# outofforest/storm

Measured on AMD Instinct MI355X. Metric: GiB/s device-resident block checksum; % of MI355X HBM roofline, higher is better.
Workload: dtype u64

## Files before the change

storm_amd/csrc/commit_plan.h:

```cpp
#pragma once

#include <algorithm>
#include <atomic>
#include <cstdint>
#include <cstdlib>
#include <cstring>
#include <memory>
#include <vector>

#include "../../include/stormck.h"
#include "dispatch.h"

namespace stormck {

constexpr unsigned kMaxParts = 16;

enum class CommitError { Ok, TooMany, ParentRange, OriginAlign, Cycle, NoMem };

inline const char* commit_error_message(CommitError e) {
    switch (e) {
        case CommitError::TooMany: return "more than 2^32 dirty blocks";
        case CommitError::ParentRange: return "parent index out of range";
        case CommitError::OriginAlign: return "origin_pointer must be 8-byte aligned (Go blocks.Pointer alignment)";
        case CommitError::Cycle: return "parent links form a cycle";
// ... 193 lines not shown
    for (unsigned t = 1; t < parts; ++t)
        for (size_t l = 1; l <= max_h; ++l) pos[t][l] = pos[t - 1][l] + hist[t - 1][l];
    par(nu, [&](unsigned t, uint64_t lo, uint64_t hi) {
        std::vector<uint64_t>& ps = pos[t];
        for (uint64_t u = lo; u < hi; ++u) {
            const uint32_t i = uidx(u);
            O->order[ps[height[i]]++] = i;
        }
    });
}

template <class Par>
void commit_order(const Heights& H, Par&& par, CommitOrder* O) {
    order_level0(H, par, O);
    order_upper(H, par, O);
}

template <class Par, class Emit>
void relocate_range(stormck_dirty_block* blocks, const CommitOrder& O, uint64_t a, uint64_t b, uint64_t revision,
                    bool relocating, uint64_t* last, Par&& par, Emit&& emit) {
    if (a >= b) return;
    uint64_t before[kMaxParts + 1];
    before[0] = 0;
    unsigned parts = 0;
    if (relocating) {
        parts = par(b - a, [&](unsigned t, uint64_t lo, uint64_t hi) {
            uint64_t m = 0;
            for (uint64_t k = a + lo; k < a + hi; ++k) m += blocks[O.at(k)].birth_revision <= revision;
            before[t + 1] = m;
        });
        for (unsigned t = 0; t < parts; ++t) before[t + 1] += before[t];
    }
    const uint64_t first = *last;
    par(b - a, [&](unsigned t, uint64_t lo, uint64_t hi) {
        uint64_t addr = first + (relocating ? before[t] : 0);
        for (uint64_t k = a + lo; k < a + hi; ++k) {
            stormck_dirty_block& rec = blocks[O.at(k)];
            if (relocating && rec.birth_revision <= revision) {
                rec.address = ++addr;
                rec.birth_revision = revision + 1;
            }
            emit(k, rec);
        }
    });
    *last = first + before[parts];
}

constexpr uint64_t level0_chunk(uint64_t rest, uint64_t next) {
    return rest - std::min(next, rest) < kStreamBatch ? rest : std::min(next, rest);
}

constexpr bool commit_one_piece(uint64_t nu, uint64_t n0) { return nu > 0 && n0 <= kCommitOnePiece; }

}
```

storm_amd/csrc/dispatch.h:

```cpp
#pragma once

#include <algorithm>
#include <cstdint>
#include <cstdio>
#include <cstdlib>

#include "../../include/stormck.h"

namespace stormck {

constexpr int kU = 16;
constexpr int kQuadSpreadDepth = 4;
constexpr int kTileStripes = 16;
constexpr int kRing = 2;
constexpr int kGldsWaves = 8;
constexpr unsigned kGldsThreads = 64 * kGldsWaves;
constexpr unsigned kGldsBlocks = 16 * kGldsWaves;
constexpr int kAuxNT = 2;
constexpr uint64_t kMultiBpw = 5;
constexpr uint64_t kMultiBpwRing = 8;
constexpr uint64_t kMultiBpwWide = 16;
constexpr uint32_t kChunkPiecesWide = 128;
constexpr uint64_t kWideBatch = 128;
constexpr uint64_t kCommitWide = 256;
// ... 3 lines not shown
constexpr uint64_t kBigW = 131072;
constexpr uint64_t kBigBatch = 24576;
constexpr int kMidWaves = 2;
constexpr unsigned kThreads = 256;
constexpr uint32_t kMaxFanout = 1u << 16;
constexpr uint64_t kWideNodes = 256;
constexpr uint32_t kRingTile = 15;
constexpr int kRingPrefetch = 6;

constexpr int kSkewTiles = 8;
constexpr uint64_t kSkewMinSteps = 3584;

constexpr uint64_t kVarMinLen = 4096;
constexpr uint64_t kOrderMinBlocks = 1u << 20;

constexpr uint64_t kVarFloorPerCu = 44;
constexpr uint64_t kMidFloorPerCu = 36;
constexpr uint64_t kCommitFloorPerCu = 39;
constexpr uint64_t kAssumedCus = 256;

constexpr uint32_t kPlanRingSlots = 4;
constexpr uint64_t kPlanPipePieces = 4096;
constexpr uint64_t kPlanMultiPieces = 2034;
constexpr uint32_t kPlanOrderBuckets = 4096;
constexpr uint32_t kPlanNodeLds = 32768;
constexpr uint32_t plan_pointer_block_size(uint32_t fanout) { return (fanout * 25u + 7u) & ~7u; }

#ifdef STORMCK_PROBES
constexpr bool kProbes = true;
#else
constexpr bool kProbes = false;
#endif

struct Knobs {
    uint32_t ring_slots = kPlanRingSlots;
    bool wide16 = false;
    bool wide_multi = true;
    bool glds_var = true;
    uint64_t var_lo = 0;
    uint64_t var_min_len = kVarMinLen;
    int mid_waves = 0;
    bool big_w = true;
    uint64_t skew_min_steps = kSkewMinSteps;
    uint64_t quad_spread = 1;
    bool gather_order = true;
    bool gather_rank = false;
    bool gather_defer = false;
    bool order_idx = false;
    bool gather_contig = false;
    uint64_t commit_wide = kCommitWide;
    bool commit_multi = true;
    bool commit_midw = true;
    uint64_t commit_first = 2 * kStreamBatch, commit_growth = 3;
    int pointer_ring = 2;
    int pointer_c = 1;
    bool pointer_simd = true;
    uint64_t single_gpu_min = UINT64_MAX;
};

#ifdef STORMCK_PROBES
inline const Knobs& knobs() {
    static const Knobs once = [] {
        Knobs k;
        auto env = [](const char* name) { return std::getenv(name); };
        auto is = [&](const char* name, char c) { return env(name) && env(name)[0] == c; };
        auto num = [&](const char* name, uint64_t dflt) { return env(name) ? std::strtoull(env(name), nullptr, 10) : dflt; };
        auto integer = [&](const char* name, int dflt) { return env(name) ? std::atoi(env(name)) : dflt; };
        if (is("STORMCK_STAGE_PIPE", '0')) k.ring_slots = 0;
        k.wide16 = is("STORMCK_WIDE16", '1');
        k.wide_multi = !is("STORMCK_WIDE_MULTI", '0');
        k.glds_var = !is("STORMCK_GLDS_VAR", '0');
        k.var_lo = num("STORMCK_VAR_LO", 0);
        k.var_min_len = num("STORMCK_VAR_MIN_LEN", kVarMinLen);
        k.mid_waves = integer("STORMCK_MID_WAVES", 0);
        k.big_w = !is("STORMCK_BIG_W", '0');
        k.skew_min_steps = num("STORMCK_SKEW_MIN_STEPS", kSkewMinSteps);
        k.quad_spread = static_cast<uint64_t>(integer("STORMCK_QUAD_SPREAD", 1));
        k.gather_order = !is("STORMCK_GATHER_ORDER", '0');
        k.gather_rank = is("STORMCK_GATHER_RANK", '1');
        k.gather_defer = is("STORMCK_GATHER_DEFER", '1');
        k.order_idx = is("STORMCK_ORDER_IDX", '1');
        k.gather_contig = is("STORMCK_GATHER_CONTIG", '1');
        k.commit_multi = !is("STORMCK_COMMIT_MULTI", '0');
        k.commit_midw = !is("STORMCK_COMMIT_MIDW", '0');
        k.pointer_ring = integer("STORMCK_POINTER_RING", 2);
        k.pointer_c = integer("STORMCK_POINTER_C", 1);
        k.pointer_simd = !is("STORMCK_POINTER_SIMD", '0');
        k.single_gpu_min = num("STORMCK_SINGLE_GPU_MIN", UINT64_MAX);
        return k;
    }();
    return once;
}
inline Knobs commit_knobs() {
    Knobs k = knobs();
    if (const char* e = std::getenv("STORMCK_COMMIT_WIDE")) k.commit_wide = std::strtoull(e, nullptr, 10);
    unsigned long long f = 0, gr = 0;
    if (const char* e = std::getenv("STORMCK_COMMIT_CHUNKS"))
        if (std::sscanf(e, "%llu,%llu", &f, &gr) == 2 && f >= 1 && gr >= 1) {
            k.commit_first = f;
            k.commit_growth = gr;
        }
    return k;
}
#else
constexpr Knobs knobs() { return Knobs{}; }
constexpr Knobs commit_knobs() { return Knobs{}; }
#endif

enum class Kernel {
    Wide,
    WideMulti,
    GldsVar,
    GldsVarOrdered,
    Glds,
    GldsSkew,
    QuadSpread,
    Quad,
    PointerPc,
    TooLarge,
};

struct MultiShape {
    uint64_t bpw = 0;
    uint32_t ring = 0, chunk = 256;
    bool dbl = false;
};

struct Plan {
    Kernel kernel = Kernel::Quad;
    uint32_t grid = 0, block = kThreads;
    int waves = 0;
    bool persistent = false;
    bool simd_roles = false;
    MultiShape multi;
    uint64_t ws_bytes = 0;
    bool defer = false, idx = false, rank = false, contig = false;
};

inline Plan make_plan(Kernel k, uint64_t grid, unsigned block, int waves = 0) {
    Plan p;
    p.kernel = grid > 0x7fffffffULL ? Kernel::TooLarge : k;
    p.grid = static_cast<uint32_t>(grid);
    p.block = block;
    p.waves = waves;
    return p;
}

constexpr uint64_t busiest_cu_blocks(uint64_t n, uint64_t waves, uint64_t ncu) {
    return (((n + 16 * waves - 1) / (16 * waves)) + ncu - 1) / ncu * 16 * waves;
}
constexpr int mid_waves_for(uint64_t n, uint64_t ncu) {
    return busiest_cu_blocks(n, 1, ncu) < busiest_cu_blocks(n, 3, ncu) ? 1 : 3;
}
constexpr bool big_takes_3_waves(uint64_t n, uint64_t ncu) {
// ... 56 lines not shown
            p.rank = q.lens && persistent && k.gather_rank && n / kGldsBlocks > 0;
            p.contig = persistent && k.gather_contig;
            const uint64_t words = (uint64_t{kPlanOrderBuckets} * 3 + n + 1) & ~uint64_t{1};
            p.ws_bytes = words * 4 + n * 8 + (q.lens ? n * 4 : 0) + (p.defer ? n * 8 + 8 : 0);
        }
        return p;
    }
    int mid_waves = 0;
    if (ncu > 0 && n < kBigBatch) {
        if (k.mid_waves >= 1 && k.mid_waves <= 4) {
            if (n > 16 * ncu) mid_waves = k.mid_waves;
        } else if (k.mid_waves == 0 && n >= kMidFloorPerCu * ncu) {
            mid_waves = mid_waves_for(n, ncu);
        }
    } else if (ncu > 0 && n < kBigW && k.mid_waves == 0 && k.big_w) {
        if (big_takes_3_waves(n, ncu)) mid_waves = 3;
    }
    const bool streamable = !q.lens && !q.offs && rows16 && q.len >= 32u * kTileStripes;
    if (mid_waves > 0 && streamable)
        return make_plan(Kernel::Glds, (n + 16 * mid_waves - 1) / (16 * mid_waves), 64u * mid_waves, mid_waves);
    if (n >= kMidBatch && streamable) {
        if (n < kBigBatch)
            return make_plan(Kernel::Glds, (n + 16 * kMidWaves - 1) / (16 * kMidWaves), 64u * kMidWaves, kMidWaves);
        const uint64_t wgs = (n + kGldsBlocks - 1) / kGldsBlocks;
        if (wgs > 0x7fffffffULL) return make_plan(Kernel::TooLarge, 0, 0);
        if (ncu > 0 && wgs >= ncu && (wgs + ncu - 1) / ncu * ((q.len / 32) / kTileStripes) >= k.skew_min_steps)
            return make_plan(Kernel::GldsSkew, ncu, kGldsThreads, kGldsWaves);
        return make_plan(Kernel::Glds, wgs, kGldsThreads, kGldsWaves);
    }
    if (ncu > 0 && n <= 16 * k.quad_spread * ncu) return make_plan(Kernel::QuadSpread, (n + 15) / 16, 64);
    const uint64_t wgs = (n * 4 + kThreads - 1) / kThreads;
    return make_plan(wgs == 0 ? Kernel::TooLarge : Kernel::Quad, wgs, kThreads);
}

inline Plan plan_commit_level(uint64_t cnt, uint64_t ncu, bool glds_levels, const Knobs& k) {
    if (k.commit_midw && glds_levels && ncu > 0 && cnt >= kCommitFloorPerCu * ncu &&
        (cnt < kBigBatch || (cnt < kBigW && k.big_w && big_takes_3_waves(cnt, ncu)))) {
        const int w = cnt < kBigBatch ? mid_waves_for(cnt, ncu) : 3;
        return make_plan(Kernel::Glds, (cnt + 16 * w - 1) / (16 * w), 64u * w, w);
    }
    if (glds_levels && cnt >= kStreamBatch)
        return make_plan(Kernel::Glds, (cnt + kGldsBlocks - 1) / kGldsBlocks, kGldsThreads, kGldsWaves);
    if (cnt <= k.commit_wide) return make_plan(Kernel::Wide, cnt, kThreads);
    const MultiShape ms = multi_shape(cnt, ncu, k);
    if (k.commit_multi && ms.bpw > 0) {
        Plan p = make_plan(Kernel::WideMulti, (cnt + ms.bpw - 1) / ms.bpw, kThreads);
        p.multi = ms;
        return p;
    }
    const uint64_t wgs = (cnt * 4 + kThreads - 1) / kThreads;
    return make_plan(wgs == 0 ? Kernel::TooLarge : Kernel::Quad, wgs, kThreads);
}

inline Plan plan_pointer_level(uint64_t pm, uint32_t fanout, uint64_t ncu, const Knobs& k) {
    if (pm <= kWideNodes && plan_pointer_block_size(fanout) <= kPlanNodeLds) return make_plan(Kernel::Wide, pm, kThreads);
    if (k.pointer_ring != 0 && fanout == STORMCK_POINTERS_PER_BLOCK) {
        const uint64_t chains = (pm + 15) / 16, cus = ncu ? ncu : kAssumedCus;
        const int c = k.pointer_c == 1 || k.pointer_c == 2 || k.pointer_c == 4 ? k.pointer_c
                      : chains <= cus ? 1 : chains <= 2 * cus ? 2 : 4;
        Plan p = make_plan(Kernel::PointerPc, (chains + c - 1) / c, 128u * c, c);
        p.simd_roles = c > 1 && k.pointer_simd;
        return p;
    }
    const uint64_t wgs = (pm * 4 + kThreads - 1) / kThreads;
    return make_plan(wgs == 0 ? Kernel::TooLarge : Kernel::Quad, wgs, kThreads);
}

constexpr uint32_t kKeysPerWave = 8;
constexpr int kKeyRing = 4;
struct KeyTagsPlan {
    bool too_large = false;
    uint64_t batches = 0;
    int pieces = 0;
    bool fixed_len = false;
    uint32_t grid = 0, lds = 0;
    uint64_t tail = 0;
    uint32_t tail_grid = 0;
};

inline KeyTagsPlan plan_key_tags(uint64_t stride, uint32_t len, uint64_t n, bool offs, bool lens, unsigned base_low4) {
    KeyTagsPlan p;
    auto grid_for = [&](uint64_t threads, uint32_t* grid) {
        const uint64_t wgs = (threads + kThreads - 1) / kThreads;
        *grid = static_cast<uint32_t>(wgs);
        if (wgs == 0 || wgs > 0x7fffffffULL) p.too_large = true;
    };
    p.tail = n;
    grid_for(n, &p.tail_grid);
    if (p.too_large) return p;
    if (!offs && !lens && stride >= 16 && stride <= 256 && (stride & 15) == 0 && len <= stride && base_low4 == 0 && n >= 64) {
        p.batches = n / 64;
        p.pieces = static_cast<int>(stride / 16);
        p.fixed_len = len == stride;
        const uint64_t waves = (p.batches + kKeysPerWave - 1) / kKeysPerWave;
        p.grid = static_cast<uint32_t>((waves + 3) / 4);
        p.lds = static_cast<uint32_t>(4 * (p.pieces <= 4 ? kKeyRing : 2) * 64 * stride);
        p.tail = n - p.batches * 64;
        if (p.tail) grid_for(p.tail, &p.tail_grid);
    }
    return p;
}

}
```

storm_amd/csrc/kernels.h:

```cpp
#pragma once
#include "../../include/stormck.h"
#include "xxh64_dev.h"

namespace stormck {

typedef unsigned long long u64x2 __attribute__((ext_vector_type(2)));

#ifdef STORMCK_DEBUG_QUAD
__device__ unsigned long long g_partial_quads;
#endif

template <int K>
__device__ __forceinline__ uint64_t quad_bcast(uint64_t v) {
#ifdef STORMCK_DEBUG_QUAD
    {
        const uint64_t exec = __builtin_amdgcn_read_exec();
        const uint32_t quad = __lane_id() & ~3u;
        if (((exec >> quad) & 0xFull) != 0xFull) atomicAdd(&g_partial_quads, 1ull);
    }
#endif
    constexpr int ctrl = K | (K << 2) | (K << 4) | (K << 6);
    const int lo = __builtin_amdgcn_update_dpp(0, static_cast<int>(static_cast<uint32_t>(v)), ctrl, 0xF, 0xF, false);
    const int hi = __builtin_amdgcn_update_dpp(0, static_cast<int>(static_cast<uint32_t>(v >> 32)), ctrl, 0xF, 0xF, false);
    return (static_cast<uint64_t>(static_cast<uint32_t>(hi)) << 32) | static_cast<uint32_t>(lo);
// ... 1829 lines not shown
        out_cs[lo + first + b] = h;
        if (r.origin_pointer != STORMCK_NO_ORIGIN) {
            uint64_t* p = reinterpret_cast<uint64_t*>(arena + r.origin_pointer);
            p[0] = h;
            p[1] = r.address;
            p[2] = r.birth_revision;
            arena[r.origin_type] = r.type;
        }
    };
    if constexpr (RING > 0) {
        __shared__ uint4 ring[BPW * ring_block_pieces(RING, CP) + kRingSlackPieces];
        __shared__ uint32_t ready[pipe_max_chunks(CP)], done[1], abort_w[1];
        const PipeCtl pc{ready, done, abort_w, fault, kFaultCommitMulti, stall};
        multi_stage_hash_pipe<BPW, RING, CP, DBL>(ring, pc, nlive, src_of, emit, [](uint32_t) {});
    } else {
        __shared__ uint4 buf[BPW * kMultiPieces];
        multi_stage_hash<BPW>(buf, nlive, src_of, emit);
    }
}

template <int U>
__global__ __launch_bounds__(256) void k_commit_level(uint8_t* __restrict__ arena,
                                                       const stormck_dirty_block* __restrict__ blocks, uint64_t lo,
                                                       uint64_t cnt, uint64_t* __restrict__ out_cs) {
    const uint64_t gtid = static_cast<uint64_t>(blockIdx.x) * 256 + threadIdx.x;
    const uint64_t k = gtid >> 2;
    const uint32_t j = threadIdx.x & 3;
    const bool live = k < cnt;
    const uint64_t kk = live ? k : cnt - 1;
    const stormck_dirty_block b = blocks[lo + kk];
    const uint8_t* src = arena + b.data_offset;
    const uint32_t L = b.length;
    const uint32_t nst = L >> 5;
    uint64_t acc = acc_seed(j);
    if ((reinterpret_cast<uintptr_t>(src) & 7) == 0)
        acc = quad_stripes_aligned<U>(reinterpret_cast<const uint64_t*>(src) + j, nst, acc);
    else
        acc = quad_stripes_unaligned(src + 8 * j, nst, acc);
    const uint64_t v1 = quad_bcast<0>(acc), v2 = quad_bcast<1>(acc), v3 = quad_bcast<2>(acc), v4 = quad_bcast<3>(acc);
    if (j == 0 && live) {
        const uint64_t h0 = (L >= 32) ? converge(v1, v2, v3, v4) : kP5;
        const uint64_t h = finish_fast(h0, L, src + 32 * static_cast<uint64_t>(nst), L & 31);
        out_cs[lo + kk] = h;
        if (b.origin_pointer != STORMCK_NO_ORIGIN) {
            uint64_t* p = reinterpret_cast<uint64_t*>(arena + b.origin_pointer);
            p[0] = h;
            p[1] = b.address;
            p[2] = b.birth_revision;
            arena[b.origin_type] = b.type;
        }
    }
}

template <int T, int AUX, int WAVES>
__global__ __launch_bounds__(64 * WAVES) void k_commit_level_glds(uint8_t* __restrict__ arena,
                                                                   const stormck_dirty_block* __restrict__ blocks,
                                                                   uint64_t lo, uint64_t cnt,
                                                                   uint64_t* __restrict__ out_cs) {
    constexpr int R = 2;
    constexpr int BPW = 16 * WAVES;
    constexpr int ROW = 32 * T;
    constexpr int TILE = BPW * ROW;
    constexpr int INSTR = TILE / 1024;
    constexpr int PER_WAVE = INSTR / WAVES;
    constexpr int RW = sizeof(stormck_dirty_block) / 8;
    static_assert(INSTR % WAVES == 0, "tile must split evenly over the waves");
    __shared__ __attribute__((aligned(16))) uint8_t lds[R * TILE];
    uint64_t* rec_lds = reinterpret_cast<uint64_t*>(lds + TILE);
    static_assert(BPW * RW * 8 <= TILE, "records fit in one ring slot");

    const uint32_t tid = threadIdx.x;
    const uint32_t wave = tid >> 6, lane = tid & 63;
    const uint64_t k0 = static_cast<uint64_t>(blockIdx.x) * BPW;
    const uint32_t nrec = static_cast<uint32_t>(min<uint64_t>(BPW, cnt - k0));
    {
        const uint64_t* src = reinterpret_cast<const uint64_t*>(blocks + lo + k0);
        uint64_t w[(BPW * RW + 64 * WAVES - 1) / (64 * WAVES)];
#pragma unroll
        for (int m = 0; m < (BPW * RW + 64 * WAVES - 1) / (64 * WAVES); ++m) {
            const uint32_t q = tid + m * 64 * WAVES;
            w[m] = q < nrec * RW ? src[q] : 0;
        }
#pragma unroll
        for (int m = 0; m < (BPW * RW + 64 * WAVES - 1) / (64 * WAVES); ++m) {
            const uint32_t q = tid + m * 64 * WAVES;
            if (q < BPW * RW) rec_lds[q] = w[m];
        }
    }
    __syncthreads();
    const stormck_dirty_block* recs = reinterpret_cast<const stormck_dirty_block*>(rec_lds);

    const uint8_t* src[PER_WAVE];
    uint32_t ntl[PER_WAVE];
#pragma unroll
    for (int k = 0; k < PER_WAVE; ++k) {
        const uint32_t ii = wave * PER_WAVE + k;
        const uint32_t off = ii * 1024 + lane * 16;
        const uint32_t bb = off / ROW, q = (off % ROW) / 16;
        const uint32_t piece = (q + glds_rot<T>(bb)) % (2 * T);
        const bool plive = bb < nrec;
        const stormck_dirty_block& r = recs[plive ? bb : 0];
        src[k] = arena + r.data_offset + piece * 16;
        ntl[k] = plive ? (r.length >> 5) / T : 0;
    }
    const uint32_t b = tid >> 2, j = tid & 3;
    const uint64_t kb = k0 + b;
    const bool live = b < nrec;
    const stormck_dirty_block rec = recs[live ? b : 0];
    const uint32_t L = rec.length, nst = L >> 5;
    const uint32_t my_tiles = live ? nst / T : 0;
    uint32_t wg_tiles = my_tiles;
#pragma unroll
    for (int m = 32; m >= 1; m >>= 1) wg_tiles = max(wg_tiles, static_cast<uint32_t>(__shfl_xor(static_cast<int>(wg_tiles), m)));
    uint32_t* red = reinterpret_cast<uint32_t*>(lds);
    if (lane == 0) red[wave] = wg_tiles;
    __syncthreads();
    wg_tiles = 0;
    for (int w = 0; w < WAVES; ++w) wg_tiles = max(wg_tiles, red[w]);
    __syncthreads();

    const uint32_t rot = glds_rot<T>(b);
    uint64_t acc = acc_seed(j);
#if defined(__HIP_DEVICE_COMPILE__)
#define STORMCK_GLDS_ISSUE_MASKED(T_, SLOT)                                                              \
    do {                                                                                              \
        uint8_t* dst_ = lds + (SLOT) * TILE + wave * PER_WAVE * 1024;                                \
        _Pragma("unroll") for (int k_ = 0; k_ < PER_WAVE; ++k_) if ((T_) < ntl[k_])                   \
            __builtin_amdgcn_global_load_lds(src[k_] + static_cast<uint64_t>(T_) * ROW, dst_ + k_ * 1024, \
                                             16, 0, AUX);                                             \
    } while (0)
#else
#define STORMCK_GLDS_ISSUE_MASKED(T_, SLOT) do { } while (0)
#endif
    if (wg_tiles > 0) STORMCK_GLDS_ISSUE_MASKED(0u, 0);
    for (uint32_t t = 0; t < wg_tiles; ++t) {
        wait_vmcnt<0>();
        __builtin_amdgcn_s_barrier();
        if (t + 1 < wg_tiles) STORMCK_GLDS_ISSUE_MASKED(t + 1, (t + 1) & 1);
        if (t < my_tiles) {
            const uint8_t* row = lds + (t & 1) * TILE + b * ROW + (j & 1) * 8;
#pragma unroll
            for (int s = 0; s < T; ++s) {
                const uint32_t q = (2 * s + (j >> 1) + 2 * T - rot) % (2 * T);
                acc = round(acc, *reinterpret_cast<const uint64_t*>(row + q * 16));
            }
        }
    }
#undef STORMCK_GLDS_ISSUE_MASKED
    const uint8_t* bsrc = arena + rec.data_offset;
    for (uint32_t s = my_tiles * T; s < nst; ++s) acc = round(acc, reinterpret_cast<const uint64_t*>(bsrc)[4 * s + j]);
    const uint64_t v1 = quad_bcast<0>(acc), v2 = quad_bcast<1>(acc), v3 = quad_bcast<2>(acc), v4 = quad_bcast<3>(acc);
    if (j == 0 && live) {
        const uint64_t h0 = (L >= 32) ? converge(v1, v2, v3, v4) : kP5;
        const uint64_t h = finish_fast(h0, L, bsrc + 32 * static_cast<uint64_t>(nst), L & 31);
        out_cs[lo + kb] = h;
        if (rec.origin_pointer != STORMCK_NO_ORIGIN) {
            uint64_t* p = reinterpret_cast<uint64_t*>(arena + rec.origin_pointer);
            p[0] = h;
            p[1] = rec.address;
            p[2] = rec.birth_revision;
            arena[rec.origin_type] = rec.type;
        }
    }
}

__device__ __forceinline__ uint64_t ld64_any(const uint8_t* p, bool aligned) {
    return aligned ? *reinterpret_cast<const uint64_t*>(p) : ld64_unaligned(p);
}

template <bool OFFS, bool LENS>
__global__ __launch_bounds__(256) void k_key_tags(const uint8_t* __restrict__ keys, uint64_t stride,
                                                   const uint64_t* __restrict__ offs, const uint32_t* __restrict__ lens,
                                                   uint32_t len, uint64_t n, uint64_t* __restrict__ out) {
    const uint64_t i = static_cast<uint64_t>(blockIdx.x) * 256 + threadIdx.x;
    if (i >= n) return;
    const uint8_t* p = keys + (OFFS ? offs[i] : i * stride);
    const uint32_t L = LENS ? lens[i] : len;
    const bool al = (reinterpret_cast<uintptr_t>(p) & 7) == 0;
    const uint32_t nst = L >> 5;
    uint64_t h;
    if (L >= 32) {
        uint64_t v1 = kV1, v2 = kV2, v3 = kV3, v4 = kV4;
        for (uint32_t s = 0; s < nst; ++s) {
            const uint8_t* q = p + 32 * s;
            v1 = round(v1, ld64_any(q, al));
            v2 = round(v2, ld64_any(q + 8, al));
            v3 = round(v3, ld64_any(q + 16, al));
            v4 = round(v4, ld64_any(q + 24, al));
        }
        h = converge(v1, v2, v3, v4);
    } else {
        h = kP5;
    }
    out[i] = finish_fast(h, L, p + 32 * nst, L & 31);
}

template <int AUX, int P, int RING, int PW, int KLEN = 0, int SM = 0>
__global__ __launch_bounds__(256) void k_key_tags_ring(const uint8_t* __restrict__ keys, uint32_t len_rt,
                                                        uint64_t batches, uint64_t* __restrict__ out) {
    static_assert(RING >= 2 && PW >= RING, "ring");
    static_assert(KLEN >= 0 && KLEN <= 16 * P, "key length within the stride");
    const uint32_t len = KLEN > 0 ? static_cast<uint32_t>(KLEN) : len_rt;
    constexpr uint32_t kStride = 16 * P, kRegion = 64 * kStride;
    extern __shared__ __attribute__((aligned(16))) uint8_t dyn_lds[];
    const uint32_t wave = threadIdx.x >> 6, lane = threadIdx.x & 63;
    uint8_t* buf = dyn_lds + wave * RING * kRegion;
    const uint64_t b0 = (static_cast<uint64_t>(blockIdx.x) * 4 + wave) * PW;
    if (b0 >= batches) return;
    const uint32_t nb = static_cast<uint32_t>(batches - b0 < PW ? batches - b0 : PW);
    const uint32_t nst = len >> 5, rem = len & 31;
#if defined(__HIP_DEVICE_COMPILE__)
#define STORMCK_RING_ISSUE(I)                                                                              \
    do {                                                                                                  \
        const uint8_t* s_ = keys + (b0 + (I)) * kRegion + lane * 16;                                      \
        uint8_t* d_ = buf + ((I) % RING) * kRegion;                                                       \
        _Pragma("unroll") for (int p_ = 0; p_ < P; ++p_)                                                  \
// ... 145 lines not shown
```

storm_amd/csrc/stormck.hip:

```cpp
#include <hip/hip_runtime.h>

#include <algorithm>
#include <chrono>
#include <cstdlib>
#include <atomic>
#include <condition_variable>
#include <cstdio>
#include <cstring>
#include <memory>
#include <mutex>
#include <string>
#include <system_error>
#include <functional>
#include <thread>
#include <type_traits>
#include <vector>

#include <dlfcn.h>
#include <fcntl.h>
#include <pthread.h>
#include <sched.h>
#include <sys/uio.h>
#include <unistd.h>

// ... 518 lines not shown
        t0 = last = std::chrono::steady_clock::now();
    }
    void mark(const char* phase) {
        if (!on) return;
        const auto now = std::chrono::steady_clock::now();
        char buf[96];
        std::snprintf(buf, sizeof buf, " %s=%.3fms", phase, std::chrono::duration<double, std::milli>(now - last).count());
        log += buf;
        last = now;
    }
    ~PhaseTimer() {
        if (!on) return;
        const auto now = std::chrono::steady_clock::now();
        std::fprintf(stderr, "[stormck] %s total=%.3fms%s\n", what,
                     std::chrono::duration<double, std::milli>(now - t0).count(), log.c_str());
    }
};

__global__ void k_init_result(uint64_t* r, uint64_t n) {
    if (threadIdx.x == 0) {
        r[0] = n;
        r[1] = 0;
    }
}

constexpr uint64_t kChunkBytes = 256ULL << 20;
constexpr int kStages = 2;

struct Stage {
    hipStream_t stream = nullptr;
    hipEvent_t done = nullptr;
    hipEvent_t ready = nullptr;
    uint8_t* pinned = nullptr;
    uint8_t* d_data = nullptr;
    uint32_t* d_lens = nullptr;
    uint64_t* d_offs = nullptr;
    uint64_t* d_out = nullptr;
    uint64_t* h_out = nullptr;
    uint64_t* d_expected = nullptr;
    uint64_t* d_result = nullptr;
    uint64_t* h_result = nullptr;
    uint64_t first = 0, count = 0;
    bool busy = false;
};

struct DeviceCtx {
    std::mutex mu;
    int device = -1;
    bool ready = false;
    Stage st[kStages];
    stormck_dirty_block* commit_rec = nullptr;
    uint64_t* commit_cs = nullptr;
    uint64_t commit_n = 0;
};

std::mutex g_ctx_mu;
std::vector<std::unique_ptr<DeviceCtx>> g_ctx;

int get_ctx(DeviceCtx** out) {
    int rc = device_check();
    if (rc) return rc;
    int dev = 0;
    HIP_TRY(hipGetDevice(&dev));
    rc = fault_table_ready(dev);
    if (rc) return rc;
    std::lock_guard<std::mutex> g(g_ctx_mu);
    if (g_ctx.size() <= static_cast<size_t>(dev)) g_ctx.resize(dev + 1);
    if (!g_ctx[dev]) {
        g_ctx[dev].reset(new DeviceCtx());
        g_ctx[dev]->device = dev;
    }
    *out = g_ctx[dev].get();
    return STORMCK_OK;
}

int ensure_ready(DeviceCtx* c) {
    if (c->ready) return STORMCK_OK;
    for (Stage& s : c->st) {
        HIP_TRY(hipStreamCreateWithFlags(&s.stream, hipStreamNonBlocking));
        HIP_TRY(hipEventCreateWithFlags(&s.done, hipEventDisableTiming));
        HIP_TRY(hipEventCreateWithFlags(&s.ready, hipEventDisableTiming | hipEventBlockingSync));
        HIP_TRY(hipHostMalloc(reinterpret_cast<void**>(&s.pinned), kChunkBytes, hipHostMallocDefault));
        HIP_TRY(hipMalloc(&s.d_data, kChunkBytes));
        const uint64_t maxb = kChunkBytes / 8;
        HIP_TRY(hipMalloc(&s.d_lens, maxb * 4));
        HIP_TRY(hipMalloc(&s.d_offs, maxb * 8));
        HIP_TRY(hipMalloc(&s.d_out, maxb * 8));
        HIP_TRY(hipMalloc(&s.d_expected, maxb * 8));
        HIP_TRY(hipHostMalloc(reinterpret_cast<void**>(&s.h_out), maxb * 8, hipHostMallocDefault));
        HIP_TRY(hipMalloc(&s.d_result, 16));
        HIP_TRY(hipHostMalloc(reinterpret_cast<void**>(&s.h_result), 16, hipHostMallocDefault));
    }
    c->ready = true;
    return STORMCK_OK;
}

void release_ctx(DeviceCtx* c) {
    if (!c || (!c->ready && !c->commit_rec)) return;
    int prev = 0;
    (void)hipGetDevice(&prev);
    (void)hipSetDevice(c->device);
    for (Stage& s : c->st) {
        if (s.stream) (void)hipStreamSynchronize(s.stream);
        (void)hipFree(s.d_data);
        (void)hipFree(s.d_lens);
        (void)hipFree(s.d_offs);
        (void)hipFree(s.d_out);
        (void)hipFree(s.d_expected);
        (void)hipFree(s.d_result);
        (void)hipHostFree(s.pinned);
        (void)hipHostFree(s.h_out);
        (void)hipHostFree(s.h_result);
        if (s.done) (void)hipEventDestroy(s.done);
        if (s.ready) (void)hipEventDestroy(s.ready);
        if (s.stream) (void)hipStreamDestroy(s.stream);
        s = Stage();
    }
    c->ready = false;
    if (c->commit_rec) (void)hipHostFree(c->commit_rec);
    if (c->commit_cs) (void)hipHostFree(c->commit_cs);
    c->commit_rec = nullptr;
    c->commit_cs = nullptr;
    c->commit_n = 0;
    (void)hipSetDevice(prev);
}

bool host_readable(const void* p, uint64_t bytes) {
    const uint8_t* b = static_cast<const uint8_t*>(p);
    uint8_t got[2];
    iovec local = {got, 2};
    iovec remote[2] = {{const_cast<uint8_t*>(b), 1}, {const_cast<uint8_t*>(b + (bytes ? bytes - 1 : 0)), 1}};
    const ssize_t r = process_vm_readv(getpid(), &local, 1, remote, 2, 0);
    if (r == 2) return true;
    if (r >= 0 || errno == EFAULT) return false;
    static std::mutex mu;
    static int fds[2] = {-1, -1};
    std::lock_guard<std::mutex> g(mu);
    if (fds[0] < 0 && pipe2(fds, O_NONBLOCK | O_CLOEXEC) != 0) return true;
    for (const uint8_t* q : {b, b + (bytes ? bytes - 1 : 0)}) {
        if (write(fds[1], q, 1) != 1) return errno != EFAULT;
        uint8_t sink = 0;
        (void)!read(fds[0], &sink, 1);
    }
    return true;
}

enum class Mem {
    kPageable,
    kPinned,
    kMapped,
    kDevice,
    kUnreadable,
};
constexpr int kRegSlots = 16;
std::mutex g_reg_mu;
std::atomic<uintptr_t> g_reg_lo[kRegSlots], g_reg_hi[kRegSlots];
std::atomic<int> g_reg_n{0};

bool in_registered(const void* p, uint64_t bytes) {
    const int n = g_reg_n.load(std::memory_order_acquire);
    const uintptr_t x = reinterpret_cast<uintptr_t>(p);
    for (int k = 0; k < n; ++k) {
        const uintptr_t lo = g_reg_lo[k].load(std::memory_order_acquire);
        const uintptr_t hi = g_reg_hi[k].load(std::memory_order_acquire);
        if (lo && x >= lo && x < hi && bytes <= hi - x) return true;
    }
    return false;
}

void reg_add(void* p, uint64_t bytes) {
    std::lock_guard<std::mutex> g(g_reg_mu);
    for (int k = 0; k < kRegSlots; ++k)
        if (g_reg_lo[k].load(std::memory_order_relaxed) == 0) {
            g_reg_hi[k].store(reinterpret_cast<uintptr_t>(p) + bytes, std::memory_order_release);
            g_reg_lo[k].store(reinterpret_cast<uintptr_t>(p), std::memory_order_release);
            if (k >= g_reg_n.load(std::memory_order_relaxed)) g_reg_n.store(k + 1, std::memory_order_release);
// ... 941 lines not shown
        if (p.pieces <= 4)
            with_int<1, 2, 3, 4>(p.pieces, [&](auto P) {
                with_consts([&](auto FIXED) {
                    hipLaunchKernelGGL((k_key_tags_ring<kAuxNT, STORMCK_V(P), kKeyRing, kKeysPerWave,
                                                        STORMCK_V(FIXED) ? 16 * STORMCK_V(P) : 0, kKeyStore>),
                                       dim3(p.grid), dim3(kThreads), p.lds, st, k, len, p.batches, d_out);
                }, p.fixed_len);
            });
        else
            hipLaunchKernelGGL(k_key_tags_lds<kAuxNT>, dim3(p.grid), dim3(kThreads), p.lds, st, k,
                               static_cast<uint32_t>(stride), len, p.batches, kKeysPerWave, d_out);
        HIP_TRY(hipGetLastError());
        if (p.tail == 0) return STORMCK_OK;
        k += p.batches * 64 * stride;
        d_out += p.batches * 64;
    }
    with_consts([&](auto OFFS, auto LENS) {
        hipLaunchKernelGGL((k_key_tags<STORMCK_V(OFFS), STORMCK_V(LENS)>), dim3(p.tail_grid), dim3(kThreads), 0, st, k, stride,
                           d_offsets, d_lens, len, p.tail, d_out);
    }, d_offsets != nullptr, d_lens != nullptr);
    HIP_TRY(hipGetLastError());
    return STORMCK_OK;
}


}

namespace {

struct PoolPar {
    unsigned cap;
    uint64_t grain;
    template <class F>
    unsigned operator()(uint64_t count, F&& fn) const {
        if (cap <= 1 || count < grain) {
            fn(0u, uint64_t{0}, count);
            return 1;
        }
        ForkJoin& fj = ForkJoin::get();
        const unsigned nt = static_cast<unsigned>(std::min<uint64_t>({cap, kMaxParts, fj.size(), count / grain + 1}));
        fj.run(nt, [&](unsigned t) { fn(t, count * t / nt, count * (t + 1) / nt); });
        return nt;
    }
};
PoolPar plan_par(uint32_t threads = 0) { return {threads ? threads : kMaxParts, 16384}; }
PoolPar stage_par(uint32_t threads = 0) { return {threads ? std::min(threads, 8u) : 8u, 8192}; }

int commit_forest(const stormck_dirty_block* blocks, uint64_t n, uint64_t revision, uint32_t threads, Heights* H) {
    const CommitError e = commit_heights(blocks, n, revision, plan_par(threads), H);
    if (e == CommitError::Ok) return STORMCK_OK;
    return fail(e == CommitError::NoMem ? STORMCK_ENOMEM : STORMCK_EINVAL, commit_error_message(e));
}

int commit_device_run(void* d_arena, stormck_dirty_block* blocks, const Heights& H, uint64_t revision,
                      uint64_t* last_allocated_block, uint64_t* out_checksums, void* stream, PhaseTimer& pt) {
    ForkJoin& fj = ForkJoin::get();
    const uint64_t n = H.n, nu = H.n_upper, n0 = H.n0();
    const bool glds_levels =
        (reinterpret_cast<uintptr_t>(d_arena) & 15) == 0 && !H.data_off16 && H.longest > knobs().var_min_len;

    DeviceCtx* c = nullptr;
    int rc = get_ctx(&c);
    if (rc) return rc;
    std::lock_guard<std::mutex> g(c->mu);
    rc = ensure_ready(c);
    if (rc) return rc;
    if (c->commit_n < n) {
        if (c->commit_rec) (void)hipHostFree(c->commit_rec);
        if (c->commit_cs) (void)hipHostFree(c->commit_cs);
        c->commit_rec = nullptr;
        c->commit_cs = nullptr;
        c->commit_n = 0;
        HIP_TRY(hipHostMalloc(reinterpret_cast<void**>(&c->commit_rec), n * sizeof(stormck_dirty_block),
                              hipHostMallocCoherent));
        HIP_TRY(hipHostMalloc(reinterpret_cast<void**>(&c->commit_cs), n * 8, hipHostMallocCoherent));
        c->commit_n = n;
    }
    stormck_dirty_block* d_blocks = nullptr;
    uint64_t* d_cs = nullptr;
    HIP_TRY(hipHostGetDevicePointer(reinterpret_cast<void**>(&d_blocks), c->commit_rec, 0));
    HIP_TRY(hipHostGetDevicePointer(reinterpret_cast<void**>(&d_cs), c->commit_cs, 0));
    pt.mark("ctx");

    CommitOrder O;
    if (!H.prefix0()) {
        order_level0(H, plan_par(), &O);
        pt.mark("order0");
    }
    const std::vector<uint32_t>& order = O.order;

    hipStream_t st = static_cast<hipStream_t>(stream);
    const Knobs kn = commit_knobs();
    const uint64_t ncu = cu_count();
    uint8_t* arena = static_cast<uint8_t*>(d_arena);
    auto launch_level = [&](uint64_t lo, uint64_t cnt) -> int {
        const Plan p = plan_commit_level(cnt, ncu, glds_levels, kn);
        const dim3 grid(p.grid), block(p.block);
        switch (p.kernel) {
            case Kernel::TooLarge:
                return fail(STORMCK_EINVAL, "level too large");
            case Kernel::Glds:
                with_int<1, 3, kGldsWaves>(p.waves, [&](auto W) {
                    hipLaunchKernelGGL((k_commit_level_glds<kTileStripes, kAuxNT, STORMCK_V(W)>), grid, block, 0, st, arena,
                                       d_blocks, lo, cnt, d_cs);
                });
                break;
            case Kernel::Wide:
                hipLaunchKernelGGL(k_commit_level_wide, grid, block, 0, st, arena, d_blocks, lo, d_cs);
                break;
            case Kernel::WideMulti: {
                const int mrc = launch_wide_multi(p.multi, st, [&](auto BPW, auto RING, auto CHUNK, auto DBL, uint32_t* fault,
                                                                   uint32_t stall) {
                    hipLaunchKernelGGL((k_commit_level_multi<STORMCK_V(BPW), STORMCK_V(RING), STORMCK_V(CHUNK), STORMCK_V(DBL)>),
                                       grid, block, 0, st, arena, d_blocks, lo, cnt, d_cs, fault, stall);
                });
                if (mrc) return mrc;
                break;
            }
            default:
                hipLaunchKernelGGL(k_commit_level<kU>, grid, block, 0, st, arena, d_blocks, lo, cnt, d_cs);
        }
        HIP_TRY(hipGetLastError());
        return STORMCK_OK;
    };
    uint64_t last = *last_allocated_block;
    auto stage_records = [&](uint64_t a, uint64_t b) {
        stormck_dirty_block* rec = c->commit_rec;
        if (!H.relocating && order.empty()) {
            par_copy(reinterpret_cast<uint8_t*>(rec + a), reinterpret_cast<const uint8_t*>(blocks + a),
                     (b - a) * sizeof(stormck_dirty_block), 1ULL << 20);
            return;
        }
        relocate_range(blocks, O, a, b, revision, H.relocating != 0, &last, stage_par(),
                       [rec](uint64_t k, const stormck_dirty_block& r) { rec[k] = r; });
    };
    struct Back {
        uint64_t lo, cnt;
        hipEvent_t hashed;
    };
    std::vector<Back> back;
    auto send_back = [&](uint64_t lo, uint64_t cnt) -> int {
        back.push_back({lo, cnt, nullptr});
        HIP_TRY(hipEventCreateWithFlags(&back.back().hashed, hipEventDisableTiming));
        HIP_TRY(hipEventRecord(back.back().hashed, st));
        return STORMCK_OK;
    };
    auto run = [&]() -> int {
        const bool one_piece = commit_one_piece(nu, n0);
        uint64_t unsent = 0;
        for (uint64_t lo = 0, cnt, next = kn.commit_first; lo < n0; lo += cnt, next = cnt * kn.commit_growth) {
            cnt = level0_chunk(n0 - lo, next);
            stage_records(lo, lo + cnt);
            int e = launch_level(lo, cnt);
            if (e) return e;
            if (!one_piece) {
                e = send_back(lo, cnt);
                if (e) return e;
                unsent = lo + cnt;
            }
        }
        pt.mark("level0_issue");
        if (nu == 0) return STORMCK_OK;
        order_upper(H, plan_par(), &O);
        pt.mark("order_upper");
        stage_records(n0, n);
        int e = STORMCK_OK;
        for (uint32_t l = 1; l <= H.max_h; ++l) {
            const uint64_t lo = O.level_start[l], cnt = O.level_start[l + 1] - lo;
            if (cnt == 0) continue;
            e = launch_level(lo, cnt);
            if (e) return e;
        }
        return send_back(unsent, n - unsent);
    };
    rc = run();
    *last_allocated_block = last;
    if (rc == STORMCK_OK) {
        for (const Back& x : back) {
            if (hipEventSynchronize(x.hashed) != hipSuccess) {
                rc = fail(STORMCK_EHIP, "commit: checksum copy-back failed");
                break;
            }
            rc = take_fault(c->device, st);
            if (rc) break;
            const unsigned tn = static_cast<unsigned>(std::min<uint64_t>({8, fj.size(), x.cnt / 65536 + 1}));
            fj.run(tn, [&](unsigned t) {
                const uint64_t lo = x.lo + x.cnt * t / tn, hi = x.lo + x.cnt * (t + 1) / tn;
                if (order.empty()) {
                    std::memcpy(out_checksums + lo, c->commit_cs + lo, (hi - lo) * 8);
                } else {
                    for (uint64_t k = lo; k < hi; ++k) out_checksums[order[k]] = c->commit_cs[k];
                }
            });
        }
    }
    const hipError_t s1 = hipStreamSynchronize(st);
    for (Back& x : back) (void)hipEventDestroy(x.hashed);
    if (rc == STORMCK_OK && s1 != hipSuccess) rc = fail(STORMCK_EHIP, std::string("commit: ") + hipGetErrorString(s1));
    if (rc == STORMCK_OK) rc = take_fault(c->device, st);
    pt.mark("device");
    return rc;
}

}

namespace {

constexpr uint64_t kHostMinBytesPerThread = 256 * 1024;
constexpr double kHostLevelUs = 10.0;
constexpr double kDevCallUs = 10.0;
constexpr double kDevLevelUs = 6.0;
constexpr double kDevChainBytesPerUs = 1600.0;
constexpr double kDevBatchCallUs = 16.0;
constexpr double kStageCopyBytesPerUs = 55000.0;
constexpr double kSplitChunkUs = 8.0;
constexpr double kSplitMinClaimBytes = 1 << 20;
constexpr double kSplitDmaBytes = 32 << 20;
constexpr double kSplitGain = 0.95;
constexpr double kSplitGainCached = 0.8;
constexpr double kHostOnlyUs = 10.0;
constexpr double kSplitMinSaveUs = 30.0;

constexpr double kPriorHostThreadX4 = 48000.0;
constexpr double kPriorHostThread = 24000.0;
constexpr double kPriorHostMemory = 180000.0;
constexpr double kPriorLinkPinned = 55000.0;
constexpr double kPriorLinkPageable = 55000.0;
constexpr double kPriorLinkInplace = 50000.0;
constexpr double kPriorDeviceLatencyUs = 150.0;
constexpr double kLearnWeight = 0.25;
constexpr uint64_t kLearnMinHostBytes = 8ULL << 20;
constexpr uint64_t kLearnMinLinkBytes = 64ULL << 20;
constexpr uint64_t kHostCacheBytes = 64ULL << 20;

enum class Link { kPinned, kPageable, kInplace };

class RouteModel {
  public:
    static RouteModel& get() {
        static RouteModel m;
        return m;
    }
    stormck_route_rates now() {
        std::lock_guard<std::mutex> g(mu_);
        return r_;
    }
    double host_thread() const { return ht_.load(std::memory_order_relaxed); }
    void set(const stormck_route_rates* r, bool freeze) {
        std::lock_guard<std::mutex> g(mu_);
        r_ = r ? *r : priors();
        r_.observations = 0;
        frozen_ = freeze;
// ... 693 lines not shown
    if (p.leg == STORMCK_LEG_DEVICE) {
        const double t0 = now_us();
        int cur = 0;
        HIP_TRY(hipGetDevice(&cur));
        rc = devs.size() == 1 && devs[0] == cur
                 ? host_pipeline(hb, &mem, out, expected, first_bad, n_bad)
                 : host_pipeline_multi(base, stride, lens, len, n, out, expected, first_bad, n_bad, devs.data(),
                                       static_cast<int>(devs.size()));
        if (rc == STORMCK_OK)
            RouteModel::get().learn_link(pinned ? Link::kPinned : Link::kPageable, hb.bytes / devs.size(),
                                         now_us() - t0 - kDevBatchCallUs -
                                             static_cast<double>(hb.longest) / kDevChainBytesPerUs);
        return rc;
    }
    const unsigned pl = host_threads_for(hb.bytes, nt);
    if (p.leg == STORMCK_LEG_SPLIT)
        return batch_legs(hb, out, expected, first_bad, n_bad, devs, pl, STORMCK_SPLIT_BALANCED, nullptr,
                          mem == Mem::kMapped);
    return batch_host_leg(hb, out, expected, first_bad, n_bad, pl);
}

int split_entry(const void* base, uint64_t stride, const uint32_t* lens, uint32_t len, uint64_t n, uint64_t* out,
                const uint64_t* expected, uint64_t* first_bad, uint64_t* n_bad, const int* devices, int n_devices,
                uint32_t host_threads, uint64_t device_blocks, uint64_t* device_done) {
    if (device_done) *device_done = 0;
    HostBatch hb;
    int rc = host_batch(base, stride, lens, len, n, expected ? static_cast<const void*>(expected) : out, "null argument",
                        true, &hb);
    if (rc) return rc;
    rc = device_check();
    if (rc) return rc;
    std::vector<int> devs;
    rc = split_devices(devices, n_devices, &devs);
    if (rc) return rc;
    if (n == 0) return empty_batch(first_bad, n_bad);
    const Mem mem = classify(base, hb.extent);
    if (mem == Mem::kDevice || mem == Mem::kUnreadable) return not_host_memory(mem);
    if (mem == Mem::kPageable)
        return fail(STORMCK_EINVAL, "the split leg needs pinned or registered host memory (stormck_host_register)");
    return batch_legs(hb, out, expected, first_bad, n_bad, devs, host_threads_for(hb.bytes, pool_threads(host_threads)),
                      device_blocks, device_done, mem == Mem::kMapped);
}

}

extern "C" {

int stormck_commit_device(void* d_arena, stormck_dirty_block* blocks, uint64_t n, uint64_t revision,
                          uint64_t* last_allocated_block, uint64_t* out_checksums, void* stream) {
    static_assert(sizeof(stormck_dirty_block) == 56, "stormck_dirty_block ABI");
    if (n == 0) return STORMCK_OK;
    if (!d_arena || !blocks || !last_allocated_block || !out_checksums) return fail(STORMCK_EINVAL, "null argument");
    PhaseTimer pt("commit");
    Heights H;
    const int rc = commit_forest(blocks, n, revision, 0, &H);
    if (rc) return rc;
    pt.mark("heights");
    return commit_device_run(d_arena, blocks, H, revision, last_allocated_block, out_checksums, stream, pt);
}

int stormck_commit_host(void* arena, stormck_dirty_block* blocks, uint64_t n, uint64_t revision,
                        uint64_t* last_allocated_block, uint64_t* out_checksums, uint32_t threads) {
    if (n == 0) return STORMCK_OK;
    if (!arena || !blocks || !last_allocated_block || !out_checksums) return fail(STORMCK_EINVAL, "null argument");
    Heights H;
    const int rc = commit_forest(blocks, n, revision, threads, &H);
    if (rc) return rc;
    return commit_host_run(static_cast<uint8_t*>(arena), blocks, H, revision, last_allocated_block, out_checksums, threads,
                           {}, 0, nullptr);
}

int stormck_commit_split(void* arena, stormck_dirty_block* blocks, uint64_t n, uint64_t revision,
                         uint64_t* last_allocated_block, uint64_t* out_checksums, const int* devices, int n_devices,
                         uint32_t host_threads, uint64_t device_leaves, uint64_t* device_done) {
    if (device_done) *device_done = 0;
    if (n == 0) return STORMCK_OK;
    if (!arena || !blocks || !last_allocated_block || !out_checksums) return fail(STORMCK_EINVAL, "null argument");
    int rc = device_check();
    if (rc) return rc;
    std::vector<int> devs;
    rc = split_devices(devices, n_devices, &devs);
    if (rc) return rc;
    const Mem mem = classify(arena, 1);
    if (mem != Mem::kMapped)
        return fail(STORMCK_EINVAL, "the split commit needs the arena registered (stormck_host_register)");
    Heights H;
    rc = commit_forest(blocks, n, revision, host_threads, &H);
    if (rc) return rc;
    return commit_host_run(static_cast<uint8_t*>(arena), blocks, H, revision, last_allocated_block, out_checksums,
                           host_threads, devs, device_leaves, device_done);
}

int stormck_commit(void* arena, stormck_dirty_block* blocks, uint64_t n, uint64_t revision,
                   uint64_t* last_allocated_block, uint64_t* out_checksums, void* stream, uint32_t host_threads,
                   uint32_t* leg_used) {
    if (leg_used) *leg_used = STORMCK_LEG_NONE;
    if (n == 0) return STORMCK_OK;
    if (!arena || !blocks || !last_allocated_block || !out_checksums) return fail(STORMCK_EINVAL, "null argument");
    int rc = device_check();
    if (rc) return rc;
    const Mem mem = classify(arena, 1);
    if (mem == Mem::kDevice) {
        if (leg_used) *leg_used = STORMCK_LEG_DEVICE;
        return stormck_commit_device(arena, blocks, n, revision, last_allocated_block, out_checksums, stream);
    }
    if (mem == Mem::kUnreadable) return not_host_memory(mem);
    const bool registered = mem == Mem::kMapped;
    {
        const double bound = kHostOnlyUs * RouteModel::get().host_thread();
        uint64_t total = 0;
        for (uint64_t i = 0; i < n && static_cast<double>(total) < bound; ++i) total += blocks[i].length;
// ... 223 lines not shown
```

Before: 6645.

## Speculatively hash leading leaf blocks on device while host computes commit heights

Before the host computes the forest heights, the commit path stages a prefix of contiguous aligned leaf records and launches a hash-only level kernel on them. If the heights confirm those records form the level-0 prefix, the main run skips re-hashing them and only launches a scatter kernel to write origin pointers. Otherwise the speculative result is dropped. It also caches the device pointers and completion events in the context instead of recreating them each call, and skips a redundant fault check after draining. This adds complexity and may waste device work when the speculation is discarded.

```diff
diff --git a/storm_amd/csrc/commit_plan.h b/storm_amd/csrc/commit_plan.h
--- a/storm_amd/csrc/commit_plan.h
+++ b/storm_amd/csrc/commit_plan.h
@@ -269,4 +269,33 @@
 
 constexpr bool commit_one_piece(uint64_t nu, uint64_t n0) { return nu > 0 && n0 <= kCommitOnePiece; }
 
-}
+
+template <class Par>
+uint64_t spec_stage(const stormck_dirty_block* blocks, uint64_t cap, stormck_dirty_block* dst, Par&& par) {
+    struct Part {
+        uint64_t hi, stop;
+    } part[kMaxParts];
+    const unsigned parts = par(cap, [&](unsigned t, uint64_t lo, uint64_t hi) {
+        uint64_t i = lo;
+        for (; i < hi; ++i) {
+            const stormck_dirty_block& b = blocks[i];
+            if (b.type != STORMCK_LEAF_BLOCK || (b.data_offset & 15) != 0) break;
+            dst[i] = b;
+        }
+        part[t] = {hi, i};
+    });
+    uint64_t end = 0;
+    for (unsigned t = 0; t < parts; ++t) {
+        end = part[t].stop;
+        if (part[t].stop < part[t].hi) break;
+    }
+    return end;
+}
+
+inline bool spec_keep(const Heights& H, uint64_t spec_n) { return spec_n > 0 && H.prefix0() && spec_n <= H.n0(); }
+
+constexpr uint64_t spec_next_chunk(uint64_t spec_n, uint64_t first, uint64_t growth) {
+    return spec_n >= first ? spec_n * growth : first;
+}
+
+}
diff --git a/storm_amd/csrc/dispatch.h b/storm_amd/csrc/dispatch.h
--- a/storm_amd/csrc/dispatch.h
+++ b/storm_amd/csrc/dispatch.h
@@ -79,6 +79,7 @@
     bool commit_multi = true;
     bool commit_midw = true;
     uint64_t commit_first = 2 * kStreamBatch, commit_growth = 3;
+    uint64_t commit_spec = 2 * kStreamBatch, commit_spec_min = 4 * kStreamBatch;
     int pointer_ring = 2;
     int pointer_c = 1;
     bool pointer_simd = true;
@@ -127,6 +128,10 @@
             k.commit_first = f;
             k.commit_growth = gr;
         }
+    if (const char* e = std::getenv("STORMCK_COMMIT_SPEC")) {
+        k.commit_spec = std::strtoull(e, nullptr, 10);
+        k.commit_spec_min = 1;
+    }
     return k;
 }
 #else
@@ -289,6 +294,12 @@
     return make_plan(wgs == 0 ? Kernel::TooLarge : Kernel::Quad, wgs, kThreads);
 }
 
+inline Plan plan_commit_spec(uint64_t cnt, uint64_t ncu, const Knobs& k) {
+    const Plan p = plan_commit_level(cnt, ncu, true, k);
+    if (p.kernel == Kernel::Glds) return p;
+    return make_plan(Kernel::Glds, (cnt + kGldsBlocks - 1) / kGldsBlocks, kGldsThreads, kGldsWaves);
+}
+
 inline Plan plan_pointer_level(uint64_t pm, uint32_t fanout, uint64_t ncu, const Knobs& k) {
     if (pm <= kWideNodes && plan_pointer_block_size(fanout) <= kPlanNodeLds) return make_plan(Kernel::Wide, pm, kThreads);
     if (k.pointer_ring != 0 && fanout == STORMCK_POINTERS_PER_BLOCK) {
diff --git a/storm_amd/csrc/kernels.h b/storm_amd/csrc/kernels.h
--- a/storm_amd/csrc/kernels.h
+++ b/storm_amd/csrc/kernels.h
@@ -1905,7 +1905,7 @@
     }
 }
 
-template <int T, int AUX, int WAVES>
+template <int T, int AUX, int WAVES, bool HASH_ONLY = false>
 __global__ __launch_bounds__(64 * WAVES) void k_commit_level_glds(uint8_t* __restrict__ arena,
                                                                    const stormck_dirty_block* __restrict__ blocks,
                                                                    uint64_t lo, uint64_t cnt,
@@ -2007,14 +2007,30 @@
         const uint64_t h0 = (L >= 32) ? converge(v1, v2, v3, v4) : kP5;
         const uint64_t h = finish_fast(h0, L, bsrc + 32 * static_cast<uint64_t>(nst), L & 31);
         out_cs[lo + kb] = h;
-        if (rec.origin_pointer != STORMCK_NO_ORIGIN) {
-            uint64_t* p = reinterpret_cast<uint64_t*>(arena + rec.origin_pointer);
-            p[0] = h;
-            p[1] = rec.address;
-            p[2] = rec.birth_revision;
-            arena[rec.origin_type] = rec.type;
-        }
-    }
+        if constexpr (!HASH_ONLY) {
+            if (rec.origin_pointer != STORMCK_NO_ORIGIN) {
+                uint64_t* p = reinterpret_cast<uint64_t*>(arena + rec.origin_pointer);
+                p[0] = h;
+                p[1] = rec.address;
+                p[2] = rec.birth_revision;
+                arena[rec.origin_type] = rec.type;
+            }
+        }
+    }
+}
+
+__global__ __launch_bounds__(256) void k_commit_scatter(uint8_t* __restrict__ arena,
+                                                         const stormck_dirty_block* __restrict__ blocks, uint64_t lo,
+                                                         uint64_t cnt, const uint64_t* __restrict__ cs) {
+    const uint64_t k = static_cast<uint64_t>(blockIdx.x) * 256 + threadIdx.x;
+    if (k >= cnt) return;
+    const stormck_dirty_block b = blocks[lo + k];
+    if (b.origin_pointer == STORMCK_NO_ORIGIN) return;
+    uint64_t* p = reinterpret_cast<uint64_t*>(arena + b.origin_pointer);
+    p[0] = cs[lo + k];
+    p[1] = b.address;
+    p[2] = b.birth_revision;
+    arena[b.origin_type] = b.type;
 }
 
 __device__ __forceinline__ uint64_t ld64_any(const uint8_t* p, bool aligned) {
diff --git a/storm_amd/csrc/stormck.hip b/storm_amd/csrc/stormck.hip
--- a/storm_amd/csrc/stormck.hip
+++ b/storm_amd/csrc/stormck.hip
@@ -594,6 +594,12 @@
     stormck_dirty_block* commit_rec = nullptr;
     uint64_t* commit_cs = nullptr;
     uint64_t commit_n = 0;
+    stormck_dirty_block* commit_rec_dev = nullptr;
+    uint64_t* commit_cs_dev = nullptr;
+    stormck_dirty_block* commit_spec = nullptr;
+    stormck_dirty_block* commit_spec_dev = nullptr;
+    uint64_t commit_spec_n = 0;
+    std::vector<hipEvent_t> commit_events;
 };
 
 std::mutex g_ctx_mu;
@@ -638,7 +644,7 @@
 }
 
 void release_ctx(DeviceCtx* c) {
-    if (!c || (!c->ready && !c->commit_rec)) return;
+    if (!c || (!c->ready && !c->commit_rec && !c->commit_spec && c->commit_events.empty())) return;
     int prev = 0;
     (void)hipGetDevice(&prev);
     (void)hipSetDevice(c->device);
@@ -661,9 +667,12 @@
     c->ready = false;
     if (c->commit_rec) (void)hipHostFree(c->commit_rec);
     if (c->commit_cs) (void)hipHostFree(c->commit_cs);
-    c->commit_rec = nullptr;
-    c->commit_cs = nullptr;
-    c->commit_n = 0;
+    if (c->commit_spec) (void)hipHostFree(c->commit_spec);
+    for (hipEvent_t e : c->commit_events) (void)hipEventDestroy(e);
+    c->commit_events.clear();
+    c->commit_rec = c->commit_rec_dev = c->commit_spec = c->commit_spec_dev = nullptr;
+    c->commit_cs = c->commit_cs_dev = nullptr;
+    c->commit_n = c->commit_spec_n = 0;
     (void)hipSetDevice(prev);
 }
 
@@ -1711,35 +1720,105 @@
     return fail(e == CommitError::NoMem ? STORMCK_ENOMEM : STORMCK_EINVAL, commit_error_message(e));
 }
 
+int commit_buffers(DeviceCtx* c, uint64_t n) {
+    if (c->commit_n >= n) return STORMCK_OK;
+    if (c->commit_rec) (void)hipHostFree(c->commit_rec);
+    if (c->commit_cs) (void)hipHostFree(c->commit_cs);
+    c->commit_rec = c->commit_rec_dev = nullptr;
+    c->commit_cs = c->commit_cs_dev = nullptr;
+    c->commit_n = 0;
+    HIP_TRY(hipHostMalloc(reinterpret_cast<void**>(&c->commit_rec), n * sizeof(stormck_dirty_block), hipHostMallocCoherent));
+    HIP_TRY(hipHostMalloc(reinterpret_cast<void**>(&c->commit_cs), n * 8, hipHostMallocCoherent));
+    HIP_TRY(hipHostGetDevicePointer(reinterpret_cast<void**>(&c->commit_rec_dev), c->commit_rec, 0));
+    HIP_TRY(hipHostGetDevicePointer(reinterpret_cast<void**>(&c->commit_cs_dev), c->commit_cs, 0));
+    c->commit_n = n;
+    return STORMCK_OK;
+}
+
+struct SpecRun {
+    DeviceCtx* c = nullptr;
+    std::unique_lock<std::mutex> lock;
+    uint64_t n = 0;
+};
+
+void commit_speculate(void* d_arena, const stormck_dirty_block* blocks, uint64_t n, void* stream, SpecRun* S,
+                      PhaseTimer& pt) {
+    const Knobs kn = commit_knobs();
+    if (kn.commit_spec == 0 || n < kn.commit_spec_min || n > 0xffffffffULL) return;
+    if ((reinterpret_cast<uintptr_t>(d_arena) & 15) != 0 || blocks[0].type != STORMCK_LEAF_BLOCK ||
+        blocks[0].length <= knobs().var_min_len)
+        return;
+    const uint64_t cap = std::min<uint64_t>({n, kn.commit_spec, uint64_t{1} << 24});
+    auto open = [&]() -> int {
+        DeviceCtx* c = nullptr;
+        int rc = get_ctx(&c);
+        if (rc) return rc;
+        S->lock = std::unique_lock<std::mutex>(c->mu);
+        S->c = c;
+        rc = ensure_ready(c);
+        if (rc) return rc;
+        rc = commit_buffers(c, n);
+        if (rc) return rc;
+        if (c->commit_spec_n < cap) {
+            if (c->commit_spec) (void)hipHostFree(c->commit_spec);
+            c->commit_spec = c->commit_spec_dev = nullptr;
+            c->commit_spec_n = 0;
+            HIP_TRY(hipHostMalloc(reinterpret_cast<void**>(&c->commit_spec), cap * sizeof(stormck_dirty_block),
+                                  hipHostMallocCoherent));
+            HIP_TRY(hipHostGetDevicePointer(reinterpret_cast<void**>(&c->commit_spec_dev), c->commit_spec, 0));
+            c->commit_spec_n = cap;
+        }
+        return STORMCK_OK;
+    };
+    if (open() != STORMCK_OK) {
+        if (S->lock.owns_lock()) S->lock.unlock();
+        S->c = nullptr;
+        return;
+    }
+    DeviceCtx* c = S->c;
+    const uint64_t m = spec_stage(blocks, cap, c->commit_spec, stage_par());
+    if (m == 0) return;
+    const Plan p = plan_commit_spec(m, cu_count(), kn);
+    hipStream_t st = static_cast<hipStream_t>(stream);
+    with_int<1, 3, kGldsWaves>(p.waves, [&](auto W) {
+        hipLaunchKernelGGL((k_commit_level_glds<kTileStripes, kAuxNT, STORMCK_V(W), true>), dim3(p.grid), dim3(p.block), 0, st,
+                           static_cast<uint8_t*>(d_arena), c->commit_spec_dev, uint64_t{0}, m, c->commit_cs_dev);
+    });
+    if (hipGetLastError() != hipSuccess) return;
+    S->n = m;
+    pt.mark("spec_issue");
+}
+
 int commit_device_run(void* d_arena, stormck_dirty_block* blocks, const Heights& H, uint64_t revision,
-                      uint64_t* last_allocated_block, uint64_t* out_checksums, void* stream, PhaseTimer& pt) {
+                      uint64_t* last_allocated_block, uint64_t* out_checksums, void* stream, PhaseTimer& pt,
+                      SpecRun* S = nullptr) {
     ForkJoin& fj = ForkJoin::get();
     const uint64_t n = H.n, nu = H.n_upper, n0 = H.n0();
     const bool glds_levels =
         (reinterpret_cast<uintptr_t>(d_arena) & 15) == 0 && !H.data_off16 && H.longest > knobs().var_min_len;
 
-    DeviceCtx* c = nullptr;
-    int rc = get_ctx(&c);
-    if (rc) return rc;
-    std::lock_guard<std::mutex> g(c->mu);
+    SpecRun none;
+    if (!S) S = &none;
+    int rc = STORMCK_OK;
+    if (!S->c) {
+        rc = get_ctx(&S->c);
+        if (rc) return rc;
+        S->lock = std::unique_lock<std::mutex>(S->c->mu);
+    }
+    DeviceCtx* c = S->c;
     rc = ensure_ready(c);
     if (rc) return rc;
-    if (c->commit_n < n) {
-        if (c->commit_rec) (void)hipHostFree(c->commit_rec);
-        if (c->commit_cs) (void)hipHostFree(c->commit_cs);
-        c->commit_rec = nullptr;
-        c->commit_cs = nullptr;
-        c->commit_n = 0;
-        HIP_TRY(hipHostMalloc(reinterpret_cast<void**>(&c->commit_rec), n * sizeof(stormck_dirty_block),
-                              hipHostMallocCoherent));
-        HIP_TRY(hipHostMalloc(reinterpret_cast<void**>(&c->commit_cs), n * 8, hipHostMallocCoherent));
-        c->commit_n = n;
-    }
-    stormck_dirty_block* d_blocks = nullptr;
-    uint64_t* d_cs = nullptr;
-    HIP_TRY(hipHostGetDevicePointer(reinterpret_cast<void**>(&d_blocks), c->commit_rec, 0));
-    HIP_TRY(hipHostGetDevicePointer(reinterpret_cast<void**>(&d_cs), c->commit_cs, 0));
+    rc = commit_buffers(c, n);
+    if (rc) return rc;
+    stormck_dirty_block* d_blocks = c->commit_rec_dev;
+    uint64_t* d_cs = c->commit_cs_dev;
     pt.mark("ctx");
+    hipStream_t st = static_cast<hipStream_t>(stream);
+    uint64_t spec_n = 0;
+    if (S->n) {
+        if (glds_levels && spec_keep(H, S->n)) spec_n = S->n;
+        pt.mark(spec_n ? "spec_kept" : "spec_dropped");
+    }
 
     CommitOrder O;
     if (!H.prefix0()) {
@@ -1748,7 +1827,6 @@
     }
     const std::vector<uint32_t>& order = O.order;
 
-    hipStream_t st = static_cast<hipStream_t>(stream);
     const Knobs kn = commit_knobs();
     const uint64_t ncu = cu_count();
     uint8_t* arena = static_cast<uint8_t*>(d_arena);
@@ -1798,16 +1876,38 @@
         hipEvent_t hashed;
     };
     std::vector<Back> back;
+    size_t events_used = 0;
     auto send_back = [&](uint64_t lo, uint64_t cnt) -> int {
-        back.push_back({lo, cnt, nullptr});
-        HIP_TRY(hipEventCreateWithFlags(&back.back().hashed, hipEventDisableTiming));
+        if (c->commit_events.size() == events_used) {
+            hipEvent_t e = nullptr;
+            HIP_TRY(hipEventCreateWithFlags(&e, hipEventDisableTiming));
+            c->commit_events.push_back(e);
+        }
+        back.push_back({lo, cnt, c->commit_events[events_used++]});
         HIP_TRY(hipEventRecord(back.back().hashed, st));
         return STORMCK_OK;
     };
     auto run = [&]() -> int {
         const bool one_piece = commit_one_piece(nu, n0);
         uint64_t unsent = 0;
-        for (uint64_t lo = 0, cnt, next = kn.commit_first; lo < n0; lo += cnt, next = cnt * kn.commit_growth) {
+        if (spec_n) {
+            const stormck_dirty_block* recs = c->commit_spec_dev;
+            if (H.relocating) {
+                stage_records(0, spec_n);
+                recs = d_blocks;
+            }
+            hipLaunchKernelGGL(k_commit_scatter, dim3(static_cast<uint32_t>((spec_n + 255) / 256)), dim3(256), 0, st, arena,
+                               recs, uint64_t{0}, spec_n, d_cs);
+            HIP_TRY(hipGetLastError());
+            if (!one_piece) {
+                const int e = send_back(0, spec_n);
+                if (e) return e;
+                unsent = spec_n;
+            }
+            pt.mark("scatter");
+        }
+        for (uint64_t lo = spec_n, cnt, next = spec_n ? spec_next_chunk(spec_n, kn.commit_first, kn.commit_growth) : kn.commit_first;
+             lo < n0; lo += cnt, next = cnt * kn.commit_growth) {
             cnt = level0_chunk(n0 - lo, next);
             stage_records(lo, lo + cnt);
             int e = launch_level(lo, cnt);
@@ -1834,6 +1934,7 @@
     };
     rc = run();
     *last_allocated_block = last;
+    bool drained = false;
     if (rc == STORMCK_OK) {
         for (const Back& x : back) {
             if (hipEventSynchronize(x.hashed) != hipSuccess) {
@@ -1852,11 +1953,11 @@
                 }
             });
         }
+        drained = rc == STORMCK_OK && !back.empty();
     }
     const hipError_t s1 = hipStreamSynchronize(st);
-    for (Back& x : back) (void)hipEventDestroy(x.hashed);
     if (rc == STORMCK_OK && s1 != hipSuccess) rc = fail(STORMCK_EHIP, std::string("commit: ") + hipGetErrorString(s1));
-    if (rc == STORMCK_OK) rc = take_fault(c->device, st);
+    if (rc == STORMCK_OK && !drained) rc = take_fault(c->device, st);
     pt.mark("device");
     return rc;
 }
@@ -2656,11 +2757,16 @@
     if (n == 0) return STORMCK_OK;
     if (!d_arena || !blocks || !last_allocated_block || !out_checksums) return fail(STORMCK_EINVAL, "null argument");
     PhaseTimer pt("commit");
+    SpecRun spec;
+    commit_speculate(d_arena, blocks, n, stream, &spec, pt);
     Heights H;
     const int rc = commit_forest(blocks, n, revision, 0, &H);
-    if (rc) return rc;
     pt.mark("heights");
-    return commit_device_run(d_arena, blocks, H, revision, last_allocated_block, out_checksums, stream, pt);
+    if (rc) {
+        if (spec.n) (void)hipStreamSynchronize(static_cast<hipStream_t>(stream));
+        return rc;
+    }
+    return commit_device_run(d_arena, blocks, H, revision, last_allocated_block, out_checksums, stream, pt, &spec);
 }
 
 int stormck_commit_host(void* arena, stormck_dirty_block* blocks, uint64_t n, uint64_t revision,
```

Measured after the change: 6634. About the same (-0.2%).
